# z430/keyword-spotting

Hardware: AMD Instinct MI355X
Metric: 1s 16kHz clips/sec end-to-end (wav->label) (higher is better)
Workload: dtype f32

## Files before the change

keyword-spotting_amd/csrc/kws_mfcc_f64.hip:

```cpp
#include <type_traits>

#include "kws_augment_dev.h"
#include "kws_internal.h"
#include "kws_mfcc_f64_dev.h"

namespace kws {
namespace {

constexpr int F64_MAX_WAVES = 4;
constexpr int F64_PAIRS_PER_WAVE = 4;
constexpr int F64_STAGE_MELW_MAX_NFFT = 1024;

struct F64Layout {
    size_t tw, melw, dct, edges, wave0, per_wave, total;
};
__host__ __device__ inline F64Layout f64_layout(int nfft, bool pow2, bool alias_p, int nfilt, int numcep, int n_waves) {
    const size_t nb = nfft / 2 + 1, n_tw = pow2 ? nfft / 2 : nfft;
    F64Layout l;
    l.tw = 0;
    l.melw = l.tw + 16 * n_tw;
    l.dct = l.melw + (nfft <= F64_STAGE_MELW_MAX_NFFT ? 8 * 2 * nb : 0);
    l.edges = l.dct + 8 * (size_t)numcep * nfilt;
    l.wave0 = (l.edges + 4 * (size_t)(nfilt + 2) + 15) & ~(size_t)15;
    l.per_wave = 16 * ((size_t)nfft + (alias_p ? 0 : nb)) + 8 * 128;
    l.total = l.wave0 + (size_t)n_waves * l.per_wave;
    return l;
}

struct F64Wave {
    F64Tabs tb;
    d2* X;
    d2* P;
    double* L;
};
template <bool POW2, bool ALIAS_P>
__device__ __forceinline__ F64Wave f64_stage_tables(const FrontendParams& p, const FrontendTables& t, unsigned char* smem, int nfft) {
    const int nb = nfft / 2 + 1;
    const int n_waves = blockDim.x >> 6, n_threads = blockDim.x;
    const F64Layout lay = f64_layout(nfft, POW2, ALIAS_P, p.nfilt, p.numcep, n_waves);
    const bool stage_melw = nfft <= F64_STAGE_MELW_MAX_NFFT;
    d2* tw_lds = reinterpret_cast<d2*>(smem + lay.tw);
    double* dct = reinterpret_cast<double*>(smem + lay.dct);
    int* edges = reinterpret_cast<int*>(smem + lay.edges);
    const int tid = threadIdx.x, wv = tid >> 6;
    const d2* __restrict__ twg = reinterpret_cast<const d2*>(t.tw64);
    const int n_tw = POW2 ? nfft / 2 : nfft;
    for (int i = tid; i < n_tw; i += n_threads) tw_lds[i] = twg[i];
    if (stage_melw)
        for (int i = tid; i < 2 * nb; i += n_threads) reinterpret_cast<double*>(smem + lay.melw)[i] = t.mel_w64[i];
    for (int i = tid; i < p.numcep * p.nfilt; i += n_threads) dct[i] = t.dct64[i];
    for (int i = tid; i < p.nfilt + 2; i += n_threads) edges[i] = t.mel_edges[i];
    unsigned char* mine = smem + lay.wave0 + wv * lay.per_wave;
    F64Wave w;
    w.tb.tw = tw_lds;
    w.tb.melw = stage_melw ? reinterpret_cast<const double*>(smem + lay.melw) : t.mel_w64;
    w.tb.dct = dct;
    w.tb.edges = edges;
    w.X = reinterpret_cast<d2*>(mine);
    w.P = ALIAS_P ? w.X : w.X + nfft;
    w.L = reinterpret_cast<double*>(mine + lay.per_wave - 8 * 128);
    return w;
}

template <typename T, bool POW2, int NCT>
__global__ __launch_bounds__(F64_MAX_WAVES * 64) void kws_mfcc_f64_kernel(FrontendParams p, FrontendTables t, const T* __restrict__ wav,
                                                                      float* __restrict__ out) {
    extern __shared__ __attribute__((aligned(16))) unsigned char smem64[];
    const int nfft = NCT ? NCT : p.nfft, nb = nfft / 2 + 1;
    constexpr bool ALIAS_P = POW2 && NCT > 0;
    const int n_waves = blockDim.x >> 6;
    const int tid = threadIdx.x, lane = tid & 63, wv = tid >> 6;
    const F64Wave w = f64_stage_tables<POW2, ALIAS_P>(p, t, smem64, nfft);
    __syncthreads();

    const int clip = blockIdx.y;
    const T* __restrict__ x = wav + (size_t)clip * p.n_samples;
    const int n_used = p.frame_len < nfft ? p.frame_len : nfft;
    const int n_pairs = (p.num_frames + 1) / 2;
    const int pairs_per_wg = (n_pairs + gridDim.x - 1) / gridDim.x;
    for (int pr = blockIdx.x * pairs_per_wg + wv; pr < n_pairs && pr < (blockIdx.x + 1) * pairs_per_wg; pr += n_waves) {
        const int fa = 2 * pr;
        const bool has_b = fa + 1 < p.num_frames;
        const long sa = (long)fa * p.frame_step, sb = sa + p.frame_step;
        bool nza, nzb;
        f64_load_pair<T, NCT>(p, x, sa, x, sb, has_b, w.X, nfft, n_used, lane, nza, nzb);
        spectrum_pair<POW2, NCT>(w.X, w.P, w.tb.tw, nfft, p.log2_nfft, n_used, 1.0 / (double)nfft, lane);
        float* oa = out + ((size_t)clip * p.num_frames + fa) * p.numcep;
        f64_tail<NCT ? NCT / 2 + 1 : 0>(p, w.tb, nb, w.P, w.L, nza, nzb, has_b, oa, oa + p.numcep, nullptr, lane);
    }
}

#ifndef KWS_X_REFINE_WAVES
#define KWS_X_REFINE_WAVES 12
#endif
constexpr int REFINE_WAVES = KWS_X_REFINE_WAVES;
template <typename T>
struct RaggedClip {
    const T* x;
    int len, frames, row0, pair0;
};
template <bool RAGGED, typename SrcOf>
__device__ __forceinline__ void mfcc_refine_body(const FrontendParams& p, const FrontendTables& t, float* __restrict__ out,
                                                 const RefineList& rl, SrcOf src_of) {
    extern __shared__ __attribute__((aligned(16))) unsigned char smem64[];
    constexpr int NCT = 512;
    const int tid = threadIdx.x, lane = tid & 63, wv = tid >> 6;
    const int n_waves = blockDim.x >> 6;
    const int raw = *const_cast<volatile int*>(rl.ctr);
    const int n = raw < rl.cap ? raw : rl.cap;
    if ((int)blockIdx.x < n) {
        const int n_used = p.frame_len < NCT ? p.frame_len : NCT;
        const int pairs_per_clip = (p.num_frames + 1) / 2;
        const F64Layout lay = f64_layout(NCT, true, true, p.nfilt, p.numcep, n_waves);
        d2* const X = reinterpret_cast<d2*>(smem64 + lay.wave0 + wv * lay.per_wave);
        int e = wv * gridDim.x + blockIdx.x;
        int entry = 0, clip = 0, fa = 0;
        bool has_b = false, nza = false, nzb = false;
        [[maybe_unused]] int row0 = 0;
        auto fetch = [&]() {
            entry = rl.list[e];
            const int pair = entry >> 2;
            if constexpr (RAGGED) {
                const auto rc = src_of(pair);
                FrontendParams q = p;
                q.n_samples = rc.len;
                q.num_frames = rc.frames;
                q.vec_ok = p.vec_ok && rc.len % 8 == 0;
                row0 = rc.row0;
                fa = 2 * (pair - rc.pair0);
                has_b = fa + 1 < rc.frames;
                const long sa = (long)fa * p.frame_step;
                f64_load_pair<typename std::remove_cv<typename std::remove_pointer<decltype(rc.x)>::type>::type, NCT>(
                    q, rc.x, sa, rc.x, sa + p.frame_step, has_b, X, NCT, n_used, lane, nza, nzb);
            } else {
                clip = pair / pairs_per_clip;
                fa = 2 * (pair - clip * pairs_per_clip);
                has_b = fa + 1 < p.num_frames;
#ifdef KWS_X_REFINE_SINGLE
                has_b = false;
#endif
                const auto x = src_of(clip);
                const long sa = (long)fa * p.frame_step;
                if constexpr (std::is_pointer<decltype(x)>::value) {
                    f64_load_pair<typename std::remove_cv<typename std::remove_pointer<decltype(x)>::type>::type, NCT>(
                        p, x, sa, x, sa + p.frame_step, has_b, X, NCT, n_used, lane, nza, nzb);
                } else {
                    nza = nzb = false;
                    f64_fill_pair<NCT>(p, x, sa, x, sa + p.frame_step, has_b, X, NCT, n_used, lane, nza, nzb);
                    nza = __any(nza);
                    nzb = __any(nzb);
                    wave_order();
                }
            }
        };
#ifndef KWS_X_REFINE_LATE_FETCH
        if (e < n) fetch();
#endif
        const F64Wave w = f64_stage_tables<true, true>(p, t, smem64, NCT);
        __syncthreads();
#ifdef KWS_X_REFINE_LATE_FETCH
        if (e < n) fetch();
#endif
        while (e < n) {
            spectrum_pair<true, NCT>(w.X, w.P, w.tb.tw, NCT, 9, n_used, 1.0 / (double)NCT, lane);
            float* oa;
            if constexpr (RAGGED) oa = out + (size_t)(row0 + fa) * p.numcep;
            else oa = out + ((size_t)clip * p.num_frames + fa) * p.numcep;
            f64_tail<NCT / 2 + 1>(p, w.tb, NCT / 2 + 1, w.P, w.L, nza, nzb, has_b, (entry & 1) ? oa : nullptr,
                                  (entry & 2) ? oa + p.numcep : nullptr, nullptr, lane);
            e += gridDim.x * n_waves;
            if (e < n) fetch();
        }
        __syncthreads();
    }
    int participants = n < 1 ? 1 : (n > (int)gridDim.x ? (int)gridDim.x : n);
    if ((int)blockIdx.x >= participants) return;
    if (tid == 0 && atomicAdd(&rl.ctr[6], 1) == participants - 1) {
        const int rows = rl.ctr[1];
        const unsigned long long total = ((unsigned long long)(unsigned)rl.ctr[3] << 32 | (unsigned)rl.ctr[2]) + (unsigned long long)rows;
        rl.ctr[2] = (int)(unsigned)total;
        rl.ctr[3] = (int)(unsigned)(total >> 32);
        rl.ctr[4] = rows;
        rl.ctr[6] = 0;
        rl.ctr[1] = 0;
        rl.ctr[0] = 0;
    }
}

template <typename T>
__global__ __launch_bounds__(REFINE_WAVES * 64) void kws_mfcc_refine_kernel(FrontendParams p, FrontendTables t, const T* __restrict__ wav,
                                                                         float* __restrict__ out, RefineList rl) {
    mfcc_refine_body<false>(p, t, out, rl, [&](int clip) -> const T* { return wav + (size_t)clip * p.n_samples; });
}
__global__ __launch_bounds__(REFINE_WAVES * 64) void kws_mfcc_refine_augment_kernel(FrontendParams p, FrontendTables t, AugmentArgs aug,
                                                                                 float* __restrict__ out, RefineList rl) {
    mfcc_refine_body<false>(p, t, out, rl, [&](int clip) { return aug_clip(aug, clip, p.n_samples); });
}
template <typename T>
__device__ __forceinline__ RaggedClip<T> ragged_clip_of(const T* __restrict__ pcm, const RaggedArgs& rg, int pair) {
    int lo = 0, hi = rg.R;
    while (hi - lo > 1) {
        const int mid = (lo + hi) >> 1;
        if (rg.rec[mid].pair_off <= pair) lo = mid;
        else hi = mid;
    }
    const RaggedRec rr = rg.rec[lo];
    return RaggedClip<T>{pcm + rr.start, rr.len, rr.frames, rr.frame_off, rr.pair_off};
}
__global__ __launch_bounds__(REFINE_WAVES * 64) void kws_mfcc_refine_ragged_kernel(FrontendParams p, FrontendTables t, const int16_t* __restrict__ pcm,
                                                                                float* __restrict__ out, RefineList rl, RaggedArgs rg) {
    mfcc_refine_body<true>(p, t, out, rl, [&](int pair) { return ragged_clip_of(pcm, rg, pair); });
}
__global__ __launch_bounds__(REFINE_WAVES * 64) void kws_mfcc_refine_ragged_f32_kernel(FrontendParams p, FrontendTables t, const float* __restrict__ wav,
                                                                                    float* __restrict__ out, RefineList rl, RaggedArgs rg) {
    mfcc_refine_body<true>(p, t, out, rl, [&](int pair) { return ragged_clip_of(wav, rg, pair); });
}

template <typename T>
hipError_t launch_mfcc_f64_t(hipStream_t s, const FrontendParams& p, const FrontendTables& t, const T* d_wav, int B, float* d_out) {
    const bool pow2 = p.log2_nfft > 0;
    const bool fixed = p.nfft == 512;
    int n_waves = F64_MAX_WAVES;
    while (n_waves > 1 && f64_layout(p.nfft, pow2, pow2 && fixed, p.nfilt, p.numcep, n_waves).total > 160 * 1024) --n_waves;
    const size_t lds = f64_layout(p.nfft, pow2, pow2 && fixed, p.nfilt, p.numcep, n_waves).total;
    if (lds > 160 * 1024) return hipErrorInvalidValue;
    auto kernel = fixed ? kws_mfcc_f64_kernel<T, true, 512> : pow2 ? kws_mfcc_f64_kernel<T, true, 0> : kws_mfcc_f64_kernel<T, false, 0>;
    hipError_t e = raise_lds_limit(kernel, lds);
    if (e != hipSuccess) return e;
    const int n_pairs = (p.num_frames + 1) / 2;
    const int pairs_per_wg = F64_PAIRS_PER_WAVE * n_waves;
    dim3 grid((n_pairs + pairs_per_wg - 1) / pairs_per_wg, 1);
    for (int b0 = 0; b0 < B; b0 += 65535) {
        grid.y = (B - b0 < 65535) ? (B - b0) : 65535;
        hipLaunchKernelGGL(kernel, grid, dim3(n_waves * 64), lds, s, p, t, d_wav + (size_t)b0 * p.n_samples,
                           d_out + (size_t)b0 * p.num_frames * p.numcep);
    }
    return hipGetLastError();
}

#ifndef KWS_X_REFINE_GRID
#define KWS_X_REFINE_GRID 256
#endif
constexpr int REFINE_GRID = KWS_X_REFINE_GRID;
template <typename K, typename In>
hipError_t launch_mfcc_refine_t(K kernel, hipStream_t s, const FrontendParams& p, const FrontendTables& t, const In& d_wav, float* d_out,
                                const RefineList& rl, int B) {
    const size_t lds = f64_layout(512, true, true, p.nfilt, p.numcep, REFINE_WAVES).total;
    hipError_t e = raise_lds_limit(kernel, lds);
    if (e != hipSuccess) return e;
    int grid = (B + 15) / 16;
    grid = grid < 32 ? 32 : (grid > REFINE_GRID ? REFINE_GRID : grid);
    hipLaunchKernelGGL(kernel, dim3(grid), dim3(REFINE_WAVES * 64), lds, s, p, t, d_wav, d_out, rl);
    return hipGetLastError();
}

}

hipError_t launch_mfcc_refine(hipStream_t s, const FrontendParams& p, const FrontendTables& t, const int16_t* d_wav, float* d_out,
                              const RefineList& rl, int B) {
    return launch_mfcc_refine_t(kws_mfcc_refine_kernel<int16_t>, s, p, t, d_wav, d_out, rl, B);
}
hipError_t launch_mfcc_refine(hipStream_t s, const FrontendParams& p, const FrontendTables& t, const float* d_wav, float* d_out,
                              const RefineList& rl, int B) {
    return launch_mfcc_refine_t(kws_mfcc_refine_kernel<float>, s, p, t, d_wav, d_out, rl, B);
}
hipError_t launch_mfcc_refine(hipStream_t s, const FrontendParams& p, const FrontendTables& t, const AugmentArgs& a, float* d_out,
                              const RefineList& rl, int B) {
    return launch_mfcc_refine_t(kws_mfcc_refine_augment_kernel, s, p, t, a, d_out, rl, B);
}

template <typename K, typename T>
static hipError_t launch_mfcc_refine_ragged_t(K kernel, hipStream_t s, const FrontendParams& p, const FrontendTables& t, const T* d_pcm,
                                              const RaggedArgs& rg, float* d_out, const RefineList& rl, int B) {
    const size_t lds = f64_layout(512, true, true, p.nfilt, p.numcep, REFINE_WAVES).total;
    hipError_t e = raise_lds_limit(kernel, lds);
    if (e != hipSuccess) return e;
    int grid = (B + 15) / 16;
    grid = grid < 32 ? 32 : (grid > REFINE_GRID ? REFINE_GRID : grid);
    hipLaunchKernelGGL(kernel, dim3(grid), dim3(REFINE_WAVES * 64), lds, s, p, t, d_pcm, d_out, rl, rg);
    return hipGetLastError();
}
hipError_t launch_mfcc_refine_ragged(hipStream_t s, const FrontendParams& p, const FrontendTables& t, const int16_t* d_pcm,
                                     const RaggedArgs& rg, float* d_out, const RefineList& rl, int B) {
    return launch_mfcc_refine_ragged_t(kws_mfcc_refine_ragged_kernel, s, p, t, d_pcm, rg, d_out, rl, B);
}
hipError_t launch_mfcc_refine_ragged(hipStream_t s, const FrontendParams& p, const FrontendTables& t, const float* d_wav,
                                     const RaggedArgs& rg, float* d_out, const RefineList& rl, int B) {
    return launch_mfcc_refine_ragged_t(kws_mfcc_refine_ragged_f32_kernel, s, p, t, d_wav, rg, d_out, rl, B);
}

hipError_t launch_mfcc_f64(hipStream_t s, const FrontendParams& p, const FrontendTables& t, const int16_t* d_wav, int B, float* d_out) {
    return launch_mfcc_f64_t(s, p, t, d_wav, B, d_out);
}
hipError_t launch_mfcc_f64(hipStream_t s, const FrontendParams& p, const FrontendTables& t, const float* d_wav, int B, float* d_out) {
    return launch_mfcc_f64_t(s, p, t, d_wav, B, d_out);
}

}
```

keyword-spotting_amd/csrc/kws_mfcc_f64_dev.h:

```cpp
#pragma once
#include "kws_internal.h"

namespace kws {
namespace {

typedef double d2 __attribute__((ext_vector_type(2)));

constexpr double PSF_EPS64 = 2.220446049250313e-16;

__device__ __forceinline__ float to_unit64(int16_t s) { return (float)s * (1.0f / 32768.0f); }
__device__ __forceinline__ float to_unit64(float s) { return s; }

template <typename T>
__device__ __forceinline__ float preemph_sample(const T* __restrict__ x, long m, int n_samples, float c) {
    if (m < 0 || m >= n_samples) return 0.f;
    const float cur = to_unit64(x[m]);
    return m > 0 ? __fsub_rn(cur, __fmul_rn(c, to_unit64(x[m - 1]))) : cur;
}

__device__ __forceinline__ void wave_order() {
    __builtin_amdgcn_fence(__ATOMIC_ACQ_REL, "wavefront");
    __builtin_amdgcn_wave_barrier();
}

template <int CTRL, int ROW_MASK>
__device__ __forceinline__ double dpp_shift_add_f64(double v) {
    const unsigned long long u = __builtin_bit_cast(unsigned long long, v);
    const unsigned lo = (unsigned)__builtin_amdgcn_update_dpp(0, (int)(unsigned)u, CTRL, ROW_MASK, 0xf, true);
    const unsigned hi = (unsigned)__builtin_amdgcn_update_dpp(0, (int)(unsigned)(u >> 32), CTRL, ROW_MASK, 0xf, true);
    return v + __builtin_bit_cast(double, ((unsigned long long)hi << 32) | lo);
}
__device__ __forceinline__ double wave_sum_f64(double v) {
    v = dpp_shift_add_f64<0x111, 0xf>(v);
    v = dpp_shift_add_f64<0x112, 0xf>(v);
    v = dpp_shift_add_f64<0x114, 0xf>(v);
    v = dpp_shift_add_f64<0x118, 0xf>(v);
    v = dpp_shift_add_f64<0x142, 0xa>(v);
    v = dpp_shift_add_f64<0x143, 0xc>(v);
    const unsigned long long u = __builtin_bit_cast(unsigned long long, v);
    const unsigned lo = (unsigned)__builtin_amdgcn_readlane((int)(unsigned)u, 63), hi = (unsigned)__builtin_amdgcn_readlane((int)(unsigned)(u >> 32), 63);
    return __builtin_bit_cast(double, ((unsigned long long)hi << 32) | lo);
}

template <int BOUND, typename F>
__device__ __forceinline__ void lane_loop(int lane, int n, F&& body) {
    if constexpr (BOUND > 0) {
#pragma unroll
        for (int it = 0; it < (BOUND + 63) / 64; ++it) {
            const int i = lane + 64 * it;
            if (i < n) body(i);
        }
    } else {
        for (int i = lane; i < n; i += 64) body(i);
    }
}

__device__ __forceinline__ d2 cmul64(d2 a, d2 b) {
    return d2{__builtin_fma(a.x, b.x, -(a.y * b.y)), __builtin_fma(a.x, b.y, a.y * b.x)};
}
__device__ __forceinline__ d2 add_mi64(d2 a, d2 b) { return d2{a.x + b.y, a.y - b.x}; }
__device__ __forceinline__ d2 sub_mi64(d2 a, d2 b) { return d2{a.x - b.y, a.y + b.x}; }

__device__ __forceinline__ void dft8_f64(d2 (&v)[8]) {
    constexpr double R = 0.70710678118654752440;
    const d2 b0 = v[0] + v[4], b4 = v[0] - v[4];
    const d2 b1 = v[1] + v[5], c5 = v[1] - v[5];
    const d2 b2 = v[2] + v[6], b6 = v[2] - v[6];
    const d2 b3 = v[3] + v[7], c7 = v[3] - v[7];
    const d2 b5 = d2{(c5.x + c5.y) * R, (c5.y - c5.x) * R};
    const d2 b7 = d2{(c7.y - c7.x) * R, -(c7.x + c7.y) * R};
    const d2 d0 = b0 + b2, d1 = b0 - b2, d2_ = b1 + b3, d3 = b1 - b3;
    v[0] = d0 + d2_;
    v[4] = d0 - d2_;
    v[2] = add_mi64(d1, d3);
    v[6] = sub_mi64(d1, d3);
    const d2 e0 = add_mi64(b4, b6), e1 = sub_mi64(b4, b6), e2 = b5 + b7, e3 = b5 - b7;
    v[1] = e0 + e2;
    v[5] = e0 - e2;
    v[3] = add_mi64(e1, e3);
    v[7] = sub_mi64(e1, e3);
}

__device__ __forceinline__ int sw512(int p) { return p ^ ((p >> 3) & 7); }

__device__ __forceinline__ void fft512_radix8(d2* X, const d2* tw, int lane) {
#pragma unroll
    for (int stage = 0; stage < 3; ++stage) {
        const int s = 64 >> (3 * stage);
        const int stride = 1 << (3 * stage);
        const int r = lane & (s - 1);
        const int j = ((lane - r) << 3) + r;
        d2 v[8];
#pragma unroll
        for (int m = 0; m < 8; ++m) v[m] = X[sw512(j + m * s)];
        dft8_f64(v);
        if (stage < 2) {
#pragma unroll
            for (int q = 1; q < 8; ++q) {
                const int e = r * q * stride;
                d2 w = tw[e & 255];
                if (e & 256) w = -w;
                v[q] = cmul64(v[q], w);
            }
        }
#pragma unroll
        for (int q = 0; q < 8; ++q) X[sw512(j + q * s)] = v[q];
        wave_order();
    }
}
__device__ __forceinline__ int digit_rev8x3(int k) { return sw512(((k & 7) << 6) | (k & 56) | (k >> 6)); }

template <bool POW2, int NCT>
__device__ __forceinline__ void spectrum_pair(d2* X, d2* P, const d2* tw_lds, int nfft_rt, int log2n_rt, int n_used, double scale,
                                              int lane) {
    const int nfft = NCT ? NCT : nfft_rt;
    const int log2n = NCT ? (31 - __builtin_clz(NCT ? NCT : 1)) : log2n_rt;
    const int nb = nfft / 2 + 1;
    if constexpr (POW2) {
        auto where = [&](int k) { return NCT == 512 ? digit_rev8x3(k) : (int)(__brev((unsigned)k) >> (32 - log2n)); };
        if constexpr (NCT == 512) {
#ifndef KWS_X_F64_NOFFT
            fft512_radix8(X, tw_lds, lane);
#endif
        } else {
#ifdef KWS_X_F64_NOFFT
        for (int s = nfft >> 1, step = 1; s >= nfft; s >>= 1, step <<= 1) {
#else
#ifdef KWS_X_F64_ROLLED
#pragma unroll 1
#endif
        for (int s = nfft >> 1, step = 1; s >= 1; s >>= 1, step <<= 1) {
#endif
            lane_loop<NCT / 2>(lane, nfft >> 1, [&](int i) {
                const int r = i & (s - 1);
                const int j = ((i - r) << 1) + r;
                const d2 a = X[j], b = X[j + s];
                const d2 w = tw_lds[r * step];
                const d2 d = a - b;
                X[j] = a + b;
                X[j + s] = d2{__builtin_fma(d.x, w.x, -(d.y * w.y)), __builtin_fma(d.x, w.y, d.y * w.x)};
            });
            wave_order();
        }
        }
        auto power_of = [&](const d2 z, const d2 w) {
            const double ar = 0.5 * (z.x + w.x), ai = 0.5 * (z.y - w.y);
            const double br = 0.5 * (z.y + w.y), bi = 0.5 * (w.x - z.x);
            return d2{__builtin_fma(ar, ar, ai * ai) * scale, __builtin_fma(br, br, bi * bi) * scale};
        };
        if constexpr (NCT > 0) {
            constexpr int IT = (NCT / 2 + 1 + 63) / 64;
            d2 z[IT], w[IT];
#pragma unroll
            for (int it = 0; it < IT; ++it) {
                const int k = lane + 64 * it;
                if (k < nb) {
                    z[it] = X[where(k)];
                    w[it] = X[where((nfft - k) & (nfft - 1))];
                }
            }
            wave_order();
#pragma unroll
            for (int it = 0; it < IT; ++it) {
                const int k = lane + 64 * it;
                if (k < nb) P[k] = power_of(z[it], w[it]);
            }
        } else {
            for (int k = lane; k < nb; k += 64)
                P[k] = power_of(X[where(k)], X[where((nfft - k) & (nfft - 1))]);
        }
    } else {
        for (int k = lane; k < nb; k += 64) {
            double ar = 0.0, ai = 0.0, br = 0.0, bi = 0.0;
            int idx = 0;
            for (int n = 0; n < n_used; ++n) {
                const d2 x = X[n], w = tw_lds[idx];
                ar = __builtin_fma(x.x, w.x, ar);
                ai = __builtin_fma(x.x, w.y, ai);
                br = __builtin_fma(x.y, w.x, br);
                bi = __builtin_fma(x.y, w.y, bi);
                idx += k;
                if (idx >= nfft) idx -= nfft;
            }
            P[k] = d2{__builtin_fma(ar, ar, ai * ai) * scale, __builtin_fma(br, br, bi * bi) * scale};
        }
    }
    wave_order();
}


template <int NCT, typename Src>
__device__ __forceinline__ void f64_fill_pair(const FrontendParams& p, const Src& xa, long sa, const Src& xb, long sb, bool has_b, d2* X,
                                              int nfft, int n_used, int lane, bool& nza, bool& nzb) {
    lane_loop<NCT>(lane, nfft, [&](int n) {
        double a = 0.0, b = 0.0;
        if (n < n_used) {
            a = (double)preemph_sample(xa, sa + n, p.n_samples, p.preemph);
            if (has_b) b = (double)preemph_sample(xb, sb + n, p.n_samples, p.preemph);
        }
        nza |= a != 0.0;
        nzb |= b != 0.0;
        X[NCT == 512 ? sw512(n) : n] = d2{a, b};
    });
}

template <typename T, int NCT>
__device__ __forceinline__ void f64_load_pair(const FrontendParams& p, const T* __restrict__ xa, long sa, const T* __restrict__ xb,
                                              long sb, bool has_b, d2* X, int nfft, int n_used, int lane, bool& nza, bool& nzb) {
    nza = false;
    nzb = false;
    if (sizeof(T) == 2 && p.vec_ok && (p.frame_step % 8) == 0) {
        for (int g = lane; 8 * g < nfft; g += 64) {
            double va[8], vb[8];
#pragma unroll
            for (int i = 0; i < 8; ++i) va[i] = vb[i] = 0.0;
            auto load8 = [&](const T* __restrict__ x, long s0, double (&v)[8]) {
                const long m0 = s0 + 8 * g;
                if (8 * g < n_used && m0 < p.n_samples) {
                    const uint4 raw = *reinterpret_cast<const uint4*>(x + m0);
                    const uint32_t wd[4] = {raw.x, raw.y, raw.z, raw.w};
                    float prev = m0 > 0 ? to_unit64(x[m0 - 1]) : 0.f;
#pragma unroll
                    for (int i = 0; i < 8; ++i) {
                        const float cur = to_unit64((int16_t)((wd[i >> 1] >> (16 * (i & 1))) & 0xffffu));
                        const float y = (m0 + i > 0) ? __fsub_rn(cur, __fmul_rn(p.preemph, prev)) : cur;
                        v[i] = (8 * g + i < n_used) ? (double)y : 0.0;
                        prev = cur;
                    }
                }
            };
            load8(xa, sa, va);
            if (has_b) load8(xb, sb, vb);
#pragma unroll
            for (int i = 0; i < 8; ++i) {
                nza |= va[i] != 0.0;
                nzb |= vb[i] != 0.0;
                X[NCT == 512 ? sw512(8 * g + i) : 8 * g + i] = d2{va[i], vb[i]};
            }
        }
    } else {
        f64_fill_pair<NCT>(p, xa, sa, xb, sb, has_b, X, nfft, n_used, lane, nza, nzb);
    }
    nza = __any(nza);
    nzb = __any(nzb);
    wave_order();
}

struct F64Tabs {
    const d2* tw;
    const double* melw;
    const double* dct;
    const int* edges;
};

template <int NB>
__device__ __forceinline__ void f64_tail(const FrontendParams& p, const F64Tabs& tb, int nb_rt, const d2* P, double* L, bool nza,
                                         bool nzb, bool has_b, float* __restrict__ out_a, float* __restrict__ out_b,
                                         float* lds_out_a, int lane) {
    const int nb = NB ? NB : nb_rt;
    double ea = 0.0, eb = 0.0;
    lane_loop<NB>(lane, nb, [&](int k) {
        const d2 pw = P[k];
        ea += pw.x;
        eb += pw.y;
    });
    ea = nza ? wave_sum_f64(ea) : 0.0;
    eb = nzb ? wave_sum_f64(eb) : 0.0;
    if (ea == 0.0) ea = PSF_EPS64;
    if (eb == 0.0) eb = PSF_EPS64;
#ifdef KWS_X_F64_NOTAIL
    if (out_a && lane < p.numcep) out_a[lane] = (float)(ea + eb);
    return;
#endif
    const bool split = p.nfilt <= 32;
    const int j = split ? (lane & 31) : lane;
    double fa_ = 0.0, fb_ = 0.0;
    if (j < p.nfilt) {
        const int e0 = tb.edges[j], e1 = tb.edges[j + 1], e2 = tb.edges[j + 2];
        auto edge_sum = [&](const double* __restrict__ wgt, int lo, int hi) {
            double a0 = 0.0, a1 = 0.0, a2 = 0.0, a3 = 0.0, b0 = 0.0, b1 = 0.0, b2 = 0.0, b3 = 0.0;
            int i = lo;
            for (; i + 4 <= hi; i += 4) {
                const double w0 = wgt[i], w1 = wgt[i + 1], w2 = wgt[i + 2], w3 = wgt[i + 3];
                const d2 p0 = P[i], p1 = P[i + 1], p2 = P[i + 2], p3 = P[i + 3];
                a0 = __builtin_fma(w0, p0.x, a0);
                b0 = __builtin_fma(w0, p0.y, b0);
                a1 = __builtin_fma(w1, p1.x, a1);
                b1 = __builtin_fma(w1, p1.y, b1);
                a2 = __builtin_fma(w2, p2.x, a2);
                b2 = __builtin_fma(w2, p2.y, b2);
                a3 = __builtin_fma(w3, p3.x, a3);
                b3 = __builtin_fma(w3, p3.y, b3);
            }
            for (; i < hi; ++i) {
                const double w = wgt[i];
                const d2 pw = P[i];
                a0 = __builtin_fma(w, pw.x, a0);
                b0 = __builtin_fma(w, pw.y, b0);
            }
            fa_ += (a0 + a1) + (a2 + a3);
            fb_ += (b0 + b1) + (b2 + b3);
        };
        if (!split || lane < 32) edge_sum(tb.melw, e0, e1);
        if (!split || lane >= 32) edge_sum(tb.melw + nb, e1, e2);
    }
    if (split) {
        auto other_half = [](double v) {
            const unsigned long long u = __builtin_bit_cast(unsigned long long, v);
            unsigned lo = (unsigned)u, hi = (unsigned)(u >> 32), lo2 = lo, hi2 = hi;
            asm volatile("s_nop 1\n\t"
                         "v_permlane32_swap_b32 %0, %1\n\t"
                         "v_permlane32_swap_b32 %2, %3"
                         : "+v"(lo), "+v"(lo2), "+v"(hi), "+v"(hi2));
            const bool upper = (__builtin_amdgcn_mbcnt_hi(~0u, __builtin_amdgcn_mbcnt_lo(~0u, 0u)) & 32) != 0;
            return __builtin_bit_cast(double, ((unsigned long long)(upper ? hi : hi2) << 32) | (upper ? lo : lo2));
        };
        fa_ += other_half(fa_);
        fb_ += other_half(fb_);
    }
    if (!nza) fa_ = 0.0;
    if (!nzb) fb_ = 0.0;
    double la = 0.0, lb = 0.0;
    if (lane < p.nfilt) {
        la = log(fa_ == 0.0 ? PSF_EPS64 : fa_);
        lb = log(fb_ == 0.0 ? PSF_EPS64 : fb_);
    }
    L[lane] = la;
    L[64 + lane] = lb;
    wave_order();

    const int f = lane >> 5, i = lane & 31;
    float* __restrict__ const row = f ? out_b : out_a;
    if (i < p.numcep && (f == 0 || has_b) && (row || (lds_out_a && f == 0))) {
        const double* D = tb.dct + (size_t)i * p.nfilt;
        const double* Lf = L + 64 * f;
        double acc0 = 0.0, acc1 = 0.0;
        int q = 0;
        for (; q + 8 <= p.nfilt; q += 8) {
            double dv[8], lv[8];
#pragma unroll
            for (int u = 0; u < 8; ++u) dv[u] = D[q + u], lv[u] = Lf[q + u];
#pragma unroll
            for (int u = 0; u < 8; u += 2) {
                acc0 = __builtin_fma(dv[u], lv[u], acc0);
                acc1 = __builtin_fma(dv[u + 1], lv[u + 1], acc1);
            }
        }
        for (; q < p.nfilt; ++q) acc0 = __builtin_fma(D[q], Lf[q], acc0);
        double acc = acc0 + acc1;
        if (i == 0 && p.append_energy) acc = log(f ? eb : ea);
        if (row) row[i] = (float)acc;
        if (lds_out_a && f == 0) lds_out_a[i] = (float)acc;
    }
    wave_order();
}

}
}
```

Measured before the change: 7.215 million.

## Software-pipeline refine kernel: prefetch next frame pair and stage tables via registers

The f64 refine kernel now issues the global loads for the next frame pair's PCM samples into registers before computing the current pair's spectrum and tail, then converts and stores them into LDS afterwards. Table staging into LDS is split into a register-issue phase that overlaps the first pair's load, and counter reads are hoisted to kernel entry. It also adds launch_bounds with two blocks per CU and a new grid-sizing heuristic. The aim is to hide global-memory latency in a latency-bound loop, at the cost of higher register pressure and a risk of spills under the tighter launch bound.

```diff
diff --git a/keyword-spotting_amd/csrc/kws_mfcc_f64.hip b/keyword-spotting_amd/csrc/kws_mfcc_f64.hip
--- a/keyword-spotting_amd/csrc/kws_mfcc_f64.hip
+++ b/keyword-spotting_amd/csrc/kws_mfcc_f64.hip
@@ -94,10 +94,68 @@
 #define KWS_X_REFINE_WAVES 12
 #endif
 constexpr int REFINE_WAVES = KWS_X_REFINE_WAVES;
+#define KWS_REFINE_BOUNDS __launch_bounds__(REFINE_WAVES * 64, 2)
+template <int THREADS, int COUNT, typename V>
+struct StageRegs {
+    static constexpr int IT = (COUNT + THREADS - 1) / THREADS;
+    V v[IT];
+    __device__ __forceinline__ void issue(const V* __restrict__ src, int n, int tid) {
+#pragma unroll
+        for (int k = 0; k < IT; ++k)
+            if (tid + k * THREADS < n) v[k] = src[tid + k * THREADS];
+    }
+    __device__ __forceinline__ void store(V* dst, const V* __restrict__ src, int n, int tid) const {
+#pragma unroll
+        for (int k = 0; k < IT; ++k)
+            if (tid + k * THREADS < n) dst[tid + k * THREADS] = v[k];
+        for (int i = tid + IT * THREADS; i < n; i += THREADS) dst[i] = src[i];
+    }
+};
+template <int THREADS>
+struct RefineTabRegs {
+    StageRegs<THREADS, 256, d2> tw;
+    StageRegs<THREADS, 2 * 257, double> melw;
+    StageRegs<THREADS, 512, double> dct;
+    StageRegs<THREADS, 128, int> edges;
+    __device__ __forceinline__ void issue(const FrontendParams& p, const FrontendTables& t, int tid) {
+        tw.issue(reinterpret_cast<const d2*>(t.tw64), 256, tid);
+        melw.issue(t.mel_w64, 2 * 257, tid);
+        dct.issue(t.dct64, p.numcep * p.nfilt, tid);
+        edges.issue(t.mel_edges, p.nfilt + 2, tid);
+    }
+    __device__ __forceinline__ F64Wave store(const FrontendParams& p, const FrontendTables& t, unsigned char* smem, int tid) const {
+        const F64Layout lay = f64_layout(512, true, true, p.nfilt, p.numcep, THREADS / 64);
+        F64Wave w;
+        d2* tw_lds = reinterpret_cast<d2*>(smem + lay.tw);
+        double* melw_lds = reinterpret_cast<double*>(smem + lay.melw);
+        double* dct_lds = reinterpret_cast<double*>(smem + lay.dct);
+        int* edges_lds = reinterpret_cast<int*>(smem + lay.edges);
+        tw.store(tw_lds, reinterpret_cast<const d2*>(t.tw64), 256, tid);
+        melw.store(melw_lds, t.mel_w64, 2 * 257, tid);
+        dct.store(dct_lds, t.dct64, p.numcep * p.nfilt, tid);
+        edges.store(edges_lds, t.mel_edges, p.nfilt + 2, tid);
+        unsigned char* mine = smem + lay.wave0 + (tid >> 6) * lay.per_wave;
+        w.tb.tw = tw_lds;
+        w.tb.melw = melw_lds;
+        w.tb.dct = dct_lds;
+        w.tb.edges = edges_lds;
+        w.X = reinterpret_cast<d2*>(mine);
+        w.P = w.X;
+        w.L = reinterpret_cast<double*>(mine + lay.per_wave - 8 * 128);
+        return w;
+    }
+};
 template <typename T>
 struct RaggedClip {
     const T* x;
     int len, frames, row0, pair0;
+};
+template <typename X>
+struct RefinePair {
+    X x;
+    int n_samples, frames, fa;
+    bool vec_ok;
+    size_t row;
 };
 template <bool RAGGED, typename SrcOf>
 __device__ __forceinline__ void mfcc_refine_body(const FrontendParams& p, const FrontendTables& t, float* __restrict__ out,
@@ -105,7 +163,11 @@
     extern __shared__ __attribute__((aligned(16))) unsigned char smem64[];
     constexpr int NCT = 512;
     const int tid = threadIdx.x, lane = tid & 63, wv = tid >> 6;
-    const int n_waves = blockDim.x >> 6;
+    constexpr int n_waves = REFINE_WAVES;
+    const int e0 = wv * gridDim.x + blockIdx.x;
+    const int entry0 = e0 < rl.cap ? rl.list[e0] : 0;
+    const int rows = rl.ctr[1];
+    const unsigned total_lo = (unsigned)rl.ctr[2], total_hi = (unsigned)rl.ctr[3];
     const int raw = *const_cast<volatile int*>(rl.ctr);
     const int n = raw < rl.cap ? raw : rl.cap;
     if ((int)blockIdx.x < n) {
@@ -113,71 +175,120 @@
         const int pairs_per_clip = (p.num_frames + 1) / 2;
         const F64Layout lay = f64_layout(NCT, true, true, p.nfilt, p.numcep, n_waves);
         d2* const X = reinterpret_cast<d2*>(smem64 + lay.wave0 + wv * lay.per_wave);
-        int e = wv * gridDim.x + blockIdx.x;
-        int entry = 0, clip = 0, fa = 0;
-        bool has_b = false, nza = false, nzb = false;
-        [[maybe_unused]] int row0 = 0;
-        auto fetch = [&]() {
-            entry = rl.list[e];
+        const int stride = gridDim.x * n_waves;
+        int e = e0;
+        auto locate = [&](int entry) {
             const int pair = entry >> 2;
             if constexpr (RAGGED) {
                 const auto rc = src_of(pair);
-                FrontendParams q = p;
-                q.n_samples = rc.len;
-                q.num_frames = rc.frames;
-                q.vec_ok = p.vec_ok && rc.len % 8 == 0;
-                row0 = rc.row0;
-                fa = 2 * (pair - rc.pair0);
-                has_b = fa + 1 < rc.frames;
-                const long sa = (long)fa * p.frame_step;
-                f64_load_pair<typename std::remove_cv<typename std::remove_pointer<decltype(rc.x)>::type>::type, NCT>(
-                    q, rc.x, sa, rc.x, sa + p.frame_step, has_b, X, NCT, n_used, lane, nza, nzb);
+                const int fa = 2 * (pair - rc.pair0);
+                return RefinePair<decltype(rc.x)>{rc.x, rc.len, rc.frames, fa, p.vec_ok && rc.len % 8 == 0, (size_t)(rc.row0 + fa)};
             } else {
-                clip = pair / pairs_per_clip;
-                fa = 2 * (pair - clip * pairs_per_clip);
-                has_b = fa + 1 < p.num_frames;
-#ifdef KWS_X_REFINE_SINGLE
-                has_b = false;
-#endif
-                const auto x = src_of(clip);
-                const long sa = (long)fa * p.frame_step;
-                if constexpr (std::is_pointer<decltype(x)>::value) {
-                    f64_load_pair<typename std::remove_cv<typename std::remove_pointer<decltype(x)>::type>::type, NCT>(
-                        p, x, sa, x, sa + p.frame_step, has_b, X, NCT, n_used, lane, nza, nzb);
-                } else {
-                    nza = nzb = false;
-                    f64_fill_pair<NCT>(p, x, sa, x, sa + p.frame_step, has_b, X, NCT, n_used, lane, nza, nzb);
-                    nza = __any(nza);
-                    nzb = __any(nzb);
-                    wave_order();
-                }
+                const int clip = pair / pairs_per_clip;
+                const int fa = 2 * (pair - clip * pairs_per_clip);
+                return RefinePair<decltype(src_of(clip))>{src_of(clip), p.n_samples, p.num_frames, fa, p.vec_ok != 0,
+                                                          (size_t)clip * p.num_frames + fa};
             }
         };
-#ifndef KWS_X_REFINE_LATE_FETCH
-        if (e < n) fetch();
-#endif
+        using Pair = decltype(locate(0));
+        using Sample = typename std::remove_cv<typename std::remove_pointer<decltype(Pair::x)>::type>::type;
+        constexpr bool POINTER = std::is_pointer<decltype(Pair::x)>::value;
+        auto has_b_of = [&](const Pair& j) {
+#ifdef KWS_X_REFINE_SINGLE
+            return false;
+#else
+            return j.fa + 1 < j.frames;
+#endif
+        };
+        auto params_of = [&](const Pair& j) {
+            FrontendParams q = p;
+            q.n_samples = j.n_samples;
+            q.num_frames = j.frames;
+            q.vec_ok = j.vec_ok;
+            return q;
+        };
+        bool nza = false, nzb = false;
+        auto fill = [&](const Pair& j, int lane) {
+            const long sa = (long)j.fa * p.frame_step;
+            if constexpr (POINTER) {
+                f64_load_pair<Sample, NCT>(params_of(j), j.x, sa, j.x, sa + p.frame_step, has_b_of(j), X, NCT, n_used, lane, nza, nzb);
+            } else {
+                nza = nzb = false;
+                f64_fill_pair<NCT>(p, j.x, sa, j.x, sa + p.frame_step, has_b_of(j), X, NCT, n_used, lane, nza, nzb);
+                nza = __any(nza);
+                nzb = __any(nzb);
+                wave_order();
+            }
+        };
+#ifndef KWS_X_REFINE_LOOP_STAGING
+        RefineTabRegs<n_waves * 64> tabs;
+        tabs.issue(p, t, tid);
+#endif
+        int entry = entry0;
+        int entry_next = e + stride < n ? rl.list[e + stride] : 0;
+        Pair cur{};
+        if (e < n) {
+            cur = locate(entry);
+            fill(cur, lane);
+        }
+#ifdef KWS_X_REFINE_LOOP_STAGING
         const F64Wave w = f64_stage_tables<true, true>(p, t, smem64, NCT);
-        __syncthreads();
-#ifdef KWS_X_REFINE_LATE_FETCH
-        if (e < n) fetch();
-#endif
+#else
+        const F64Wave w = tabs.store(p, t, smem64, tid);
+#endif
+        if constexpr (n_waves > 1) __syncthreads();
+        else wave_order();
         while (e < n) {
-            spectrum_pair<true, NCT>(w.X, w.P, w.tb.tw, NCT, 9, n_used, 1.0 / (double)NCT, lane);
-            float* oa;
-            if constexpr (RAGGED) oa = out + (size_t)(row0 + fa) * p.numcep;
-            else oa = out + ((size_t)clip * p.num_frames + fa) * p.numcep;
-            f64_tail<NCT / 2 + 1>(p, w.tb, NCT / 2 + 1, w.P, w.L, nza, nzb, has_b, (entry & 1) ? oa : nullptr,
-                                  (entry & 2) ? oa + p.numcep : nullptr, nullptr, lane);
-            e += gridDim.x * n_waves;
-            if (e < n) fetch();
+            const int e_next = e + stride;
+            int ln = lane;
+            asm volatile("" : "+v"(ln));
+            Pair nxt{};
+            [[maybe_unused]] F64RawPair<Sample> ahead;
+            [[maybe_unused]] bool prefetched = false;
+            int entry_after = 0;
+            if (e_next < n) {
+                nxt = locate(entry_next);
+                if (e_next + stride < n) entry_after = rl.list[e_next + stride];
+#ifndef KWS_X_REFINE_NO_PREFETCH
+                if constexpr (POINTER) {
+                    const FrontendParams q = params_of(nxt);
+                    prefetched = f64_vec_route<Sample>(q);
+                    const long sa = (long)nxt.fa * p.frame_step;
+                    if (prefetched) ahead = f64_issue_pair8(q, nxt.x, sa, nxt.x, sa + p.frame_step, has_b_of(nxt), ln, n_used);
+                }
+#endif
+            }
+            spectrum_pair<true, NCT>(w.X, w.P, w.tb.tw, NCT, 9, n_used, 1.0 / (double)NCT, ln);
+            float* const oa = out + cur.row * p.numcep;
+            f64_tail<NCT / 2 + 1>(p, w.tb, NCT / 2 + 1, w.P, w.L, nza, nzb, has_b_of(cur), (entry & 1) ? oa : nullptr,
+                                  (entry & 2) ? oa + p.numcep : nullptr, nullptr, ln);
+            e = e_next;
+            if (e < n) {
+                if constexpr (POINTER) {
+                    if (prefetched) {
+                        const long sa = (long)nxt.fa * p.frame_step;
+                        nza = nzb = false;
+                        asm volatile("" : "+v"(ln));
+                        f64_convert_pair8<Sample, NCT>(params_of(nxt), ahead, sa, sa + p.frame_step, ln, n_used, X, nza, nzb);
+                        nza = __any(nza);
+                        nzb = __any(nzb);
+                        wave_order();
+                    } else {
+                        fill(nxt, ln);
+                    }
+                } else {
+                    fill(nxt, ln);
+                }
+                cur = nxt;
+                entry = entry_next;
+                entry_next = entry_after;
+            }
         }
-        __syncthreads();
     }
     int participants = n < 1 ? 1 : (n > (int)gridDim.x ? (int)gridDim.x : n);
     if ((int)blockIdx.x >= participants) return;
     if (tid == 0 && atomicAdd(&rl.ctr[6], 1) == participants - 1) {
-        const int rows = rl.ctr[1];
-        const unsigned long long total = ((unsigned long long)(unsigned)rl.ctr[3] << 32 | (unsigned)rl.ctr[2]) + (unsigned long long)rows;
+        const unsigned long long total = ((unsigned long long)total_hi << 32 | total_lo) + (unsigned long long)rows;
         rl.ctr[2] = (int)(unsigned)total;
         rl.ctr[3] = (int)(unsigned)(total >> 32);
         rl.ctr[4] = rows;
@@ -188,11 +299,11 @@
 }
 
 template <typename T>
-__global__ __launch_bounds__(REFINE_WAVES * 64) void kws_mfcc_refine_kernel(FrontendParams p, FrontendTables t, const T* __restrict__ wav,
+__global__ KWS_REFINE_BOUNDS void kws_mfcc_refine_kernel(FrontendParams p, FrontendTables t, const T* __restrict__ wav,
                                                                          float* __restrict__ out, RefineList rl) {
     mfcc_refine_body<false>(p, t, out, rl, [&](int clip) -> const T* { return wav + (size_t)clip * p.n_samples; });
 }
-__global__ __launch_bounds__(REFINE_WAVES * 64) void kws_mfcc_refine_augment_kernel(FrontendParams p, FrontendTables t, AugmentArgs aug,
+__global__ KWS_REFINE_BOUNDS void kws_mfcc_refine_augment_kernel(FrontendParams p, FrontendTables t, AugmentArgs aug,
                                                                                  float* __restrict__ out, RefineList rl) {
     mfcc_refine_body<false>(p, t, out, rl, [&](int clip) { return aug_clip(aug, clip, p.n_samples); });
 }
@@ -207,11 +318,11 @@
     const RaggedRec rr = rg.rec[lo];
     return RaggedClip<T>{pcm + rr.start, rr.len, rr.frames, rr.frame_off, rr.pair_off};
 }
-__global__ __launch_bounds__(REFINE_WAVES * 64) void kws_mfcc_refine_ragged_kernel(FrontendParams p, FrontendTables t, const int16_t* __restrict__ pcm,
+__global__ KWS_REFINE_BOUNDS void kws_mfcc_refine_ragged_kernel(FrontendParams p, FrontendTables t, const int16_t* __restrict__ pcm,
                                                                                 float* __restrict__ out, RefineList rl, RaggedArgs rg) {
     mfcc_refine_body<true>(p, t, out, rl, [&](int pair) { return ragged_clip_of(pcm, rg, pair); });
 }
-__global__ __launch_bounds__(REFINE_WAVES * 64) void kws_mfcc_refine_ragged_f32_kernel(FrontendParams p, FrontendTables t, const float* __restrict__ wav,
+__global__ KWS_REFINE_BOUNDS void kws_mfcc_refine_ragged_f32_kernel(FrontendParams p, FrontendTables t, const float* __restrict__ wav,
                                                                                     float* __restrict__ out, RefineList rl, RaggedArgs rg) {
     mfcc_refine_body<true>(p, t, out, rl, [&](int pair) { return ragged_clip_of(wav, rg, pair); });
 }
@@ -239,18 +350,22 @@
 }
 
 #ifndef KWS_X_REFINE_GRID
-#define KWS_X_REFINE_GRID 256
+#define KWS_X_REFINE_GRID (3072 / KWS_X_REFINE_WAVES)
 #endif
 constexpr int REFINE_GRID = KWS_X_REFINE_GRID;
+inline int refine_grid(int B) {
+    int waves = (3 * B + 3) / 4;
+    waves = waves < 384 ? 384 : waves;
+    const int grid = (waves + REFINE_WAVES - 1) / REFINE_WAVES;
+    return grid > REFINE_GRID ? REFINE_GRID : grid;
+}
 template <typename K, typename In>
 hipError_t launch_mfcc_refine_t(K kernel, hipStream_t s, const FrontendParams& p, const FrontendTables& t, const In& d_wav, float* d_out,
                                 const RefineList& rl, int B) {
     const size_t lds = f64_layout(512, true, true, p.nfilt, p.numcep, REFINE_WAVES).total;
     hipError_t e = raise_lds_limit(kernel, lds);
     if (e != hipSuccess) return e;
-    int grid = (B + 15) / 16;
-    grid = grid < 32 ? 32 : (grid > REFINE_GRID ? REFINE_GRID : grid);
-    hipLaunchKernelGGL(kernel, dim3(grid), dim3(REFINE_WAVES * 64), lds, s, p, t, d_wav, d_out, rl);
+    hipLaunchKernelGGL(kernel, dim3(refine_grid(B)), dim3(REFINE_WAVES * 64), lds, s, p, t, d_wav, d_out, rl);
     return hipGetLastError();
 }
 
@@ -275,9 +390,7 @@
     const size_t lds = f64_layout(512, true, true, p.nfilt, p.numcep, REFINE_WAVES).total;
     hipError_t e = raise_lds_limit(kernel, lds);
     if (e != hipSuccess) return e;
-    int grid = (B + 15) / 16;
-    grid = grid < 32 ? 32 : (grid > REFINE_GRID ? REFINE_GRID : grid);
-    hipLaunchKernelGGL(kernel, dim3(grid), dim3(REFINE_WAVES * 64), lds, s, p, t, d_pcm, d_out, rl, rg);
+    hipLaunchKernelGGL(kernel, dim3(refine_grid(B)), dim3(REFINE_WAVES * 64), lds, s, p, t, d_pcm, d_out, rl, rg);
     return hipGetLastError();
 }
 hipError_t launch_mfcc_refine_ragged(hipStream_t s, const FrontendParams& p, const FrontendTables& t, const int16_t* d_pcm,
diff --git a/keyword-spotting_amd/csrc/kws_mfcc_f64_dev.h b/keyword-spotting_amd/csrc/kws_mfcc_f64_dev.h
--- a/keyword-spotting_amd/csrc/kws_mfcc_f64_dev.h
+++ b/keyword-spotting_amd/csrc/kws_mfcc_f64_dev.h
@@ -204,39 +204,80 @@
     });
 }
 
+template <typename T>
+struct F64Raw8 {
+    uint4 raw;
+    T before;
+    bool live;
+};
+template <typename T>
+__device__ __forceinline__ F64Raw8<T> f64_issue8(const FrontendParams& p, const T* __restrict__ x, long s0, int g, int n_used) {
+    const long m0 = s0 + 8 * g;
+    F64Raw8<T> r;
+    r.raw = uint4{0u, 0u, 0u, 0u};
+    r.before = T(0);
+    r.live = 8 * g < n_used && m0 < p.n_samples;
+    if (r.live) {
+        r.raw = *reinterpret_cast<const uint4*>(x + m0);
+        if (m0 > 0) r.before = x[m0 - 1];
+    }
+    return r;
+}
+template <typename T>
+__device__ __forceinline__ void f64_convert8(const FrontendParams& p, const F64Raw8<T>& r, long s0, int g, int n_used, double (&v)[8]) {
+    if (!r.live) return;
+    const long m0 = s0 + 8 * g;
+    const uint32_t wd[4] = {r.raw.x, r.raw.y, r.raw.z, r.raw.w};
+    float prev = m0 > 0 ? to_unit64(r.before) : 0.f;
+#pragma unroll
+    for (int i = 0; i < 8; ++i) {
+        const float cur = to_unit64((int16_t)((wd[i >> 1] >> (16 * (i & 1))) & 0xffffu));
+        const float y = (m0 + i > 0) ? __fsub_rn(cur, __fmul_rn(p.preemph, prev)) : cur;
+        v[i] = (8 * g + i < n_used) ? (double)y : 0.0;
+        prev = cur;
+    }
+}
+template <typename T>
+struct F64RawPair {
+    F64Raw8<T> a, b;
+};
+template <typename T>
+__device__ __forceinline__ F64RawPair<T> f64_issue_pair8(const FrontendParams& p, const T* __restrict__ xa, long sa,
+                                                         const T* __restrict__ xb, long sb, bool has_b, int g, int n_used) {
+    F64RawPair<T> r;
+    r.a = f64_issue8(p, xa, sa, g, n_used);
+    r.b = f64_issue8(p, xb, sb, g, has_b ? n_used : 0);
+    return r;
+}
+template <typename T, int NCT>
+__device__ __forceinline__ void f64_convert_pair8(const FrontendParams& p, const F64RawPair<T>& r, long sa, long sb, int g, int n_used,
+                                                  d2* X, bool& nza, bool& nzb) {
+    double va[8], vb[8];
+#pragma unroll
+    for (int i = 0; i < 8; ++i) va[i] = vb[i] = 0.0;
+    f64_convert8(p, r.a, sa, g, n_used, va);
+    f64_convert8(p, r.b, sb, g, n_used, vb);
+#pragma unroll
+    for (int i = 0; i < 8; ++i) {
+        nza |= va[i] != 0.0;
+        nzb |= vb[i] != 0.0;
+        X[NCT == 512 ? sw512(8 * g + i) : 8 * g + i] = d2{va[i], vb[i]};
+    }
+}
+template <typename T>
+__device__ __forceinline__ bool f64_vec_route(const FrontendParams& p) {
+    return sizeof(T) == 2 && p.vec_ok && (p.frame_step % 8) == 0;
+}
+
 template <typename T, int NCT>
 __device__ __forceinline__ void f64_load_pair(const FrontendParams& p, const T* __restrict__ xa, long sa, const T* __restrict__ xb,
                                               long sb, bool has_b, d2* X, int nfft, int n_used, int lane, bool& nza, bool& nzb) {
     nza = false;
     nzb = false;
-    if (sizeof(T) == 2 && p.vec_ok && (p.frame_step % 8) == 0) {
+    if (f64_vec_route<T>(p)) {
         for (int g = lane; 8 * g < nfft; g += 64) {
-            double va[8], vb[8];
-#pragma unroll
-            for (int i = 0; i < 8; ++i) va[i] = vb[i] = 0.0;
-            auto load8 = [&](const T* __restrict__ x, long s0, double (&v)[8]) {
-                const long m0 = s0 + 8 * g;
-                if (8 * g < n_used && m0 < p.n_samples) {
-                    const uint4 raw = *reinterpret_cast<const uint4*>(x + m0);
-                    const uint32_t wd[4] = {raw.x, raw.y, raw.z, raw.w};
-                    float prev = m0 > 0 ? to_unit64(x[m0 - 1]) : 0.f;
-#pragma unroll
-                    for (int i = 0; i < 8; ++i) {
-                        const float cur = to_unit64((int16_t)((wd[i >> 1] >> (16 * (i & 1))) & 0xffffu));
-                        const float y = (m0 + i > 0) ? __fsub_rn(cur, __fmul_rn(p.preemph, prev)) : cur;
-                        v[i] = (8 * g + i < n_used) ? (double)y : 0.0;
-                        prev = cur;
-                    }
-                }
-            };
-            load8(xa, sa, va);
-            if (has_b) load8(xb, sb, vb);
-#pragma unroll
-            for (int i = 0; i < 8; ++i) {
-                nza |= va[i] != 0.0;
-                nzb |= vb[i] != 0.0;
-                X[NCT == 512 ? sw512(8 * g + i) : 8 * g + i] = d2{va[i], vb[i]};
-            }
+            const F64RawPair<T> r = f64_issue_pair8(p, xa, sa, xb, sb, has_b, g, n_used);
+            f64_convert_pair8<T, NCT>(p, r, sa, sb, g, n_used, X, nza, nzb);
         }
     } else {
         f64_fill_pair<NCT>(p, xa, sa, xb, sb, has_b, X, nfft, n_used, lane, nza, nzb);
```

Result: no change. 7.229 million (median of 6 runs) (+0.2%).
